# mesnico/ALADIN

Measured on AMD Instinct MI355X. Metric: alignment image-text pairs/sec (BxB scores, triplet loss fwd+bwd) at B=256/GPU,R=34,T=50,D=768, higher is better.
Workload: dtype f16

## Files before the change

### aladin_amd/csrc/align_bwd.hip

```cpp
#include "../../include/aladin_hip.h"
#include "bwd_common.hpp"
#include "gemm_core.hpp"
#include "hinge_common.hpp"
#include "small_heads_common.hpp"

#define NO_GRAD 255

using BwdWs = PairWs<uint8_t>;

static size_t bwd_base_bytes(int Bi, int Bc, int T) {
  if (Bi < 1 || Bc < 1 || T < 2) return 0;
  return pair_ws_layout<uint8_t>(Bi, Bc, T - 1, nullptr, nullptr);
}

struct DenseWs { void* xm; void* xe; void* y; float* E; uint8_t* flags; void* rows; };
static size_t dense_ws_layout(const aladin_align_geom* gs, char* base, DenseWs* ws) {
  auto up = [](size_t v) { return (v + 255) / 256 * 256; };
  size_t off = 0;
  if (ws) ws->xm = base + off;
  off += up((size_t)gs->xm_bytes);
  if (ws) ws->xe = base + off;
  off += up((size_t)gs->xe_bytes + 16);
  if (ws) ws->y = base + off;
  off += up((size_t)gs->y_bytes);
// ... 99 lines not shown
      f32x16 acc;
#pragma unroll
      for (int r = 0; r < 16; ++r) acc[r] = 0.f;
      float ss = 0.f;
      if (vec) {
        for (int u = 0; u < D / 8; ++u) {
          const float4 a = *reinterpret_cast<const float4*>(xr + 8 * u + 4 * h);
          const float4 b = *reinterpret_cast<const float4*>(yr + 8 * u + 4 * h);
          ss += a.x * a.x + a.y * a.y + a.z * a.z + a.w * a.w;
          acc = __builtin_amdgcn_mfma_f32_32x32x2f32(a.x, b.x, acc, 0, 0, 0);
          acc = __builtin_amdgcn_mfma_f32_32x32x2f32(a.y, b.y, acc, 0, 0, 0);
          acc = __builtin_amdgcn_mfma_f32_32x32x2f32(a.z, b.z, acc, 0, 0, 0);
          acc = __builtin_amdgcn_mfma_f32_32x32x2f32(a.w, b.w, acc, 0, 0, 0);
        }
      } else {
        for (int k = 0; k < D; k += 2) {
          const int kk = k + h;
          const float a = kk < D ? xr[kk] : 0.f;
          const float b = kk < D ? yr[kk] : 0.f;
          ss += a * a;
          acc = __builtin_amdgcn_mfma_f32_32x32x2f32(a, b, acc, 0, 0, 0);
        }
      }
      ss += __shfl_xor(ss, 32, 64);
#pragma unroll
      for (int r = 0; r < 16; ++r) {
        const int row = cos_tile_row(r, h);
        const float inv = cos_tile_inv_norm(ss, row);
        blk[tm * 32 + row][tn * 32 + l5] = acc[r] * inv;
      }
    }
    __syncthreads();
    uint8_t* trow = table + ((int64_t)i * Bc + j) * tstride;
    for (int w = threadIdx.x; w < tstride; w += blockDim.x) {
      uint8_t res = NO_GRAD;
      if (w < Lj && Li > 0) {
        float best = blk[0][w];
        int arg = 0;
        for (int r = 1; r < Li; ++r) {
          const float v = blk[r][w];
          if (v > best) { best = v; arg = r; }
        }
        if (!(Li < Rq && best <= 0.f)) res = (uint8_t)arg;
      }
      trow[w] = res;
    }
  }
}

#define CAND_MAX 4096
#define AMBIG_MARGIN 2.2e-3f

using PairCfg = GemmCfg<2, 2, 1, 1>;
#define PAIR_STAGES 3

#ifdef ALADIN_DIAG
__device__ unsigned long long g_pair_probe[8 * 1024];
extern "C" __attribute__((visibility("default"))) int aladin_debug_read_pair_probe(unsigned long long* host_out, int n_blocks) {
  if (!host_out || n_blocks < 1 || n_blocks > 1024) { aladin_set_error("debug_read_pair_probe: bad argument"); return ALADIN_ERR_ARG; }
  if (hipMemcpyFromSymbol(host_out, HIP_SYMBOL(g_pair_probe), (size_t)n_blocks * 64) != hipSuccess) { aladin_set_error("debug_read_pair_probe: copy failed"); return ALADIN_ERR_HIP; }
  return ALADIN_OK;
}
#define PAIR_STAMP(k) do { if (threadIdx.x == 0 && blockIdx.x < 1024) g_pair_probe[8 * blockIdx.x + (k)] = __builtin_amdgcn_s_memrealtime(); } while (0)
#else
#define PAIR_STAMP(k) do { } while (0)
#endif

struct PairHinge {
  const float* S; int64_t ld; float margin; const float* val; const int* arg; float* loss; float* dS; int B; int n_pair_blocks;
  float* dST;
};
template <int SRC>
__global__ __launch_bounds__(256) void bwd_pair_argmax16_kernel(
    const half_t* __restrict__ xm, const half_t* __restrict__ xe, const half_t* __restrict__ y, int Dp, int mrows, int rem,
    int tpad, int xe_rows, int y_rows, const float* __restrict__ im, int64_t im_sb, int64_t im_sr,
    const int32_t* __restrict__ im_len, const float* __restrict__ s, int64_t s_sb, int64_t s_st,
    const int32_t* __restrict__ s_len, int Bc, int Rq, int Tq, int D, const int* __restrict__ counter,
    const int* __restrict__ pairs, uint8_t* __restrict__ table, int tstride, int x_tail,
    int y_tail, PairHinge hf, SmallFin sf) {
  if constexpr (SRC == 2) {
    if ((int)blockIdx.x >= hf.n_pair_blocks) {
      heads_small_finish_body((int)blockIdx.x - hf.n_pair_blocks, (int)gridDim.x - hf.n_pair_blocks, sf);
      return;
    }
  }
  if constexpr (SRC == 1) {
    if ((int)blockIdx.x >= hf.n_pair_blocks) {
      hinge_finish_body((int)blockIdx.x - hf.n_pair_blocks, (int)gridDim.x - hf.n_pair_blocks, hf.S, hf.ld, hf.B, hf.margin, 1,
                        hf.val, hf.arg, hf.loss, hf.dS, nullptr, nullptr, hf.dST);
      return;
    }
  }
  extern __shared__ __attribute__((aligned(16))) char pair_smem[];
  uint8_t* cand_w = reinterpret_cast<uint8_t*>(pair_smem);
  uint8_t* cand_r = cand_w + CAND_MAX;
  static_assert(2 * CAND_MAX <= PAIR_STAGES * PairCfg::STAGE_BYTES, "candidate list must fit in the ring");
  __shared__ float top_b1[2][64], top_b2[2][64];
  __shared__ int top_a1[2][64];
  __shared__ int ncand;
  __shared__ uint8_t word_amb[64], word_res[64];
  __shared__ unsigned long long word_key[64];
  const int wave = threadIdx.x >> 6, lane = threadIdx.x & 63;
  const int h = lane >> 5, l5 = lane & 31;
  const int wm = wave >> 1, wn = wave & 1;
  PAIR_STAMP(0);
  const int count = SRC != 0 ? 3 * hf.B : *counter;
  const int stride = SRC != 0 ? hf.n_pair_blocks : (int)gridDim.x;
  const int per_xcd = (count + 7) >> 3;
  for (int b = blockIdx.x; b < 8 * per_xcd; b += stride) {
    const int p = (b & 7) * per_xcd + (b >> 3);
    if (p >= count) continue;
    int i, j;
    if constexpr (SRC != 0) {
      const int q = p / 3, t = p - 3 * q, B = hf.B;
      auto row_val = [&](int v) { return SRC == 1 ? hf.val[v] : sf.st[(int64_t)v * SB_ST + 8]; };
      auto row_arg = [&](int v) { return SRC == 1 ? hf.arg[v] : __float_as_int(sf.st[(int64_t)v * SB_ST + 9]); };
      const float vr = row_val(q), vc = row_val(B + q);
      bool active;
      if (t == 0) { i = q; j = q; active = vr > 0.f || vc > 0.f; }
      else if (t == 1) { i = q; j = row_arg(q); active = vr > 0.f; }
      else {
        i = q; j = q; active = vc > 0.f;
        if (active) { i = row_arg(B + q); active = !(row_val(i) > 0.f && row_arg(i) == q); }
      }
      if (!active) continue;
    } else {
      i = pairs[p] / Bc; j = pairs[p] % Bc;
    }
    int Li = im_len[i] - 1 - x_tail; Li = Li < 0 ? 0 : (Li > Rq ? Rq : Li);
    int Lj = s_len[j] - 1 - y_tail; Lj = Lj < 0 ? 0 : (Lj > Tq ? Tq : Lj);
    __syncthreads();
    if (Li + Lj >= 0) PAIR_STAMP(1);
    if (threadIdx.x == 0) ncand = 0;
    if (threadIdx.x < 64) { word_amb[threadIdx.x] = 0; word_res[threadIdx.x] = NO_GRAD; word_key[threadIdx.x] = 0ull; }
    const int M = mrows, win = 64 - M;
    const bool side = rem > 0 && win > 0;
    int be = 0;
    if (side) be = i * rem < xe_rows - win ? i * rem : xe_rows - win;
    const int eo = side ? i * rem - be : 0;
    const int64_t yrow = (int64_t)j * tpad;
    const int64_t by = yrow < (int64_t)y_rows - 64 ? yrow : (int64_t)y_rows - 64;
    const int co = (int)(yrow - by);
    const half_t* pa1 = xm + (int64_t)i * M * Dp;
    const half_t* pa2 = side ? xe + (int64_t)be * Dp : pa1;
    f32x16 acc[1][1];
#pragma unroll
    for (int r = 0; r < 16; ++r) acc[0][0][r] = 0.f;
    uint32_t skip = 0;
    {
      const int wv = __builtin_amdgcn_readfirstlane(threadIdx.x >> 6);
      const int w0 = 32 + 8 * wv - M;
      if (w0 >= 0 && (!side || w0 + 8 <= eo || w0 >= eo + rem)) skip |= 2u;
      if (8 * wv + 8 <= co || 8 * wv >= co + tpad) skip |= 4u;
      if (32 + 8 * wv + 8 <= co || 32 + 8 * wv >= co + tpad) skip |= 8u;
    }
    gemm_mainloop<PairCfg, PAIR_STAGES>(pa1, y + by * Dp, Dp, Dp / 64, pair_smem, acc, pa2, M, skip);
    PAIR_STAMP(2);
    const int wcol = wn * 32 + l5;
    const int wd = wcol - co;
    const bool wvalid = wd >= 0 && wd < Lj && Li > 0;
    float b1 = -INFINITY, b2 = -INFINITY;
    int a1 = 255;
    auto region_of = [&](int r) {
      const int gr = wm * 32 + (r & 3) + 8 * (r >> 2) + 4 * h;
      const int d = gr - M - eo;
      const int sreg = ((unsigned)d < (unsigned)rem) ? M + d : 255;
      return gr < M ? gr : sreg;
    };
#pragma unroll
    for (int r = 0; r < 16; ++r) {
      const int reg = region_of(r);
      const float v = reg < Li ? acc[0][0][r] : -INFINITY;
      const bool first = v > b1;
      b2 = first ? b1 : (v > b2 ? v : b2);
      a1 = first ? reg : a1;
      b1 = first ? v : b1;
    }
#define TOP2_MERGE(ob1, oa1, ob2)                                                              \
    do {                                                                                       \
      if ((ob1) > b1 || ((ob1) == b1 && (oa1) < a1)) { b2 = fmaxf(b1, (ob2)); b1 = (ob1); a1 = (oa1); } \
      else b2 = fmaxf(b2, (ob1));                                                              \
    } while (0)
    {
      const float ob1 = lane_xor32(b1), ob2 = lane_xor32(b2);
      const int oa1 = lane_xor32(a1);
      TOP2_MERGE(ob1, oa1, ob2);
    }
    if (h == 0) { top_b1[wm][wcol] = b1; top_b2[wm][wcol] = b2; top_a1[wm][wcol] = a1; }
    __syncthreads();
    {
      const float ob1 = top_b1[wm ^ 1][wcol], ob2 = top_b2[wm ^ 1][wcol];
      const int oa1 = top_a1[wm ^ 1][wcol];
      TOP2_MERGE(ob1, oa1, ob2);
    }
#undef TOP2_MERGE
    if (wvalid) {
      const bool amb = (b1 - b2 < AMBIG_MARGIN) || (Li < Rq && fabsf(b1) < AMBIG_MARGIN);
      if (wm == 0 && h == 0) {
        word_amb[wd] = amb ? 1 : 0;
        word_res[wd] = (Li < Rq && b1 <= 0.f) ? NO_GRAD : (uint8_t)a1;
      }
      if (amb) {
        unsigned close = 0;
#pragma unroll
        for (int r = 0; r < 16; ++r) close |= (unsigned)(region_of(r) < Li && acc[0][0][r] > b1 - AMBIG_MARGIN) << r;
        while (close) {
          const int r = __ffs((int)close) - 1; close &= close - 1;
          const int slot = atomicAdd(&ncand, 1);
          cand_w[slot] = (uint8_t)wd;
// ... 299 lines not shown
    return ALADIN_ERR_ARG;
  }
  if (!set_ok(&im) || !set_ok(&s) || !dS || !workspace) { aladin_set_error("align_bwd: null argument"); return ALADIN_ERR_ARG; }
  if (g->Bi < 1 || g->Bc < 1 || g->R < 2 + g->x_tail || g->T < 2 + g->y_tail || g->D < 1 || ld_dS < g->Bc) { aladin_set_error("align_bwd: bad sizes"); return ALADIN_ERR_ARG; }
  if (bwd_Rq(g) > PA_MAXR - 2 || bwd_Rq(g) >= NO_GRAD || bwd_Tq(g) > PA_MAXT) { aladin_set_error("align_bwd: at most %d regions / %d words", PA_MAXR - 2, PA_MAXT); return ALADIN_ERR_UNSUPPORTED; }
  if (g->D % 4 != 0 || g->D > 1024 || im.stride_b % 4 || im.stride_r % 4 || s.stride_b % 4 || s.stride_r % 4 || ((uintptr_t)im.data & 15) || ((uintptr_t)s.data & 15)) {
    aladin_set_error("align_bwd: needs D %% 4 == 0, D <= 1024 and 16-byte aligned rows (D=%d)", g->D);
    return ALADIN_ERR_UNSUPPORTED;
  }
  if (pr.pk && g->rem && !pr.pk->xe) { aladin_set_error("align_bwd: packed operands do not belong to this problem"); return ALADIN_ERR_ARG; }
  if ((flags & ALADIN_BWD_OWN_ROW_FP16) && !(flags & ALADIN_BWD_PARTNERS_FP16)) { aladin_set_error("align_bwd: ALADIN_BWD_OWN_ROW_FP16 goes with ALADIN_BWD_PARTNERS_FP16"); return ALADIN_ERR_ARG; }
  if ((flags & ALADIN_BWD_PARTNERS_FP16) && (!pr.pk || !pr.pk->rnorm || g->split)) {
    aladin_set_error("align_bwd: ALADIN_BWD_PARTNERS_FP16 needs the forward's fp16 packed operands (xm, xe, y, rnorm) and their geometry");
    return ALADIN_ERR_ARG;
  }
  return ALADIN_OK;
}

int aladin_internal_compact_pairs(const float* dS, int64_t ld, int Bi, int Bc, int* counter, int* pairs, const char* entry, hipStream_t st) {
  if (hipMemsetAsync(counter, 0, 256, st) != hipSuccess) { aladin_set_error("%s: memset failed", entry); return ALADIN_ERR_HIP; }
  const int64_t n = (int64_t)Bi * Bc;
  int grid = (int)((n + 255) / 256); if (grid > 1024) grid = 1024;
  hipLaunchKernelGGL(bwd_compact_kernel, dim3(grid), dim3(256), 0, st, dS, ld, Bi, Bc, counter, pairs);
  return aladin_check_launch("bwd_compact_kernel");
}

template <int SRC>
static int launch_pair16(const BwdProblem& pr, const int* counter, const int* pairs, uint8_t* table, int grid, const PairHinge& hf,
                         const SmallFin& sf, const char* what) {
  const aladin_align_geom* g = pr.g;
  hipLaunchKernelGGL(bwd_pair_argmax16_kernel<SRC>, dim3(grid), dim3(256), (size_t)PAIR_STAGES * PairCfg::STAGE_BYTES, pr.st,
                     (const half_t*)pr.pk->xm, (const half_t*)pr.pk->xe, (const half_t*)pr.pk->y, g->Dp, g->mrows, g->rem, g->trows,
                     (int)g->xe_rows, (int)g->y_rows, pr.im.data, pr.im.stride_b, pr.im.stride_r, pr.im.len, pr.s.data, pr.s.stride_b,
                     pr.s.stride_r, pr.s.len, g->Bc, bwd_Rq(g), bwd_Tq(g), g->D, counter, pairs, table, table_stride(bwd_Tq(g)), g->x_tail,
                     g->y_tail, hf, sf);
  return aladin_check_launch(what);
}

static int hinge_table_check(const BwdProblem& pr, const float* S, int64_t ldS, const float* loss, const float* dS, const void* hinge_ws,
                             const void* bwd_workspace, bool small) {
  const aladin_align_geom* g = pr.g;
  if (!S || !loss || !dS || !hinge_ws || g->Bi != g->Bc || ldS < g->Bc) { aladin_set_error("hinge_argmax: bad argument"); return ALADIN_ERR_ARG; }
  if (small && g->Bc > SB_MAX) { aladin_set_error("heads_small: B = %d > %d", g->Bc, SB_MAX); return ALADIN_ERR_UNSUPPORTED; }
  if (int rc = bwd_check(pr, dS, g->Bc, nullptr, nullptr, bwd_workspace, 0)) return rc;
  if (!pr.pair16) { aladin_set_error("hinge_argmax: needs the packed fp16 operands of a class the fp16 pair kernel covers (R' <= 64, <= 64 padded words)"); return ALADIN_ERR_UNSUPPORTED; }
  return ALADIN_OK;
}
static int table_from_small_heads(const BwdProblem& pr, SmallFin sf, const BwdWs& ws) {
  const int B = pr.g->Bc, npb = (3 * B + 7) / 8 * 8;
  const PairHinge hf = {nullptr, 0, 0.f, nullptr, nullptr, nullptr, nullptr, B, npb, nullptr};
  sf.dST = (float*)ws.pairs;
  return launch_pair16<2>(pr, nullptr, nullptr, ws.table, npb + cdiv(B * B, 256), hf, sf, "bwd_pair_argmax16_kernel<small heads>");
}
static int table_from_hinge(const BwdProblem& pr, const float* S, int64_t ldS, float margin, float* loss, float* dS, void* hinge_ws,
                            const BwdWs& ws) {
  const int B = pr.g->Bc;
  if (int rc = aladin_internal_hinge_stats(S, ldS, B, margin, 1, hinge_ws, nullptr, pr.st)) return rc;
  const float* val = (const float*)hinge_ws;
  const int* arg = (const int*)(val + 2 * (size_t)B);
  int npb = (3 * B + 7) / 8 * 8; if (npb > 2048) npb = 2048;
  const int nfin = B < 1024 ? B : 1024;
  const PairHinge hf = {S, ldS, margin, val, arg, loss, dS, B, npb, (float*)ws.pairs};
  return launch_pair16<1>(pr, nullptr, nullptr, ws.table, npb + nfin, hf, SmallFin{}, "bwd_pair_argmax16_kernel<hinge>");
}

static int table_from_list(const BwdProblem& pr, const int* counter, const int* pairs, uint8_t* table) {
  const aladin_align_geom* g = pr.g;
  const int64_t n = (int64_t)g->Bi * g->Bc;
  const int grid = (int)(n < 2048 ? n : 2048);
  if (pr.pair16) return launch_pair16<0>(pr, counter, pairs, table, grid, PairHinge{}, SmallFin{}, "bwd_pair_argmax16_kernel");
  hipLaunchKernelGGL(bwd_pair_argmax_kernel, dim3(grid), dim3(256), 0, pr.st, pr.im.data, pr.im.stride_b, pr.im.stride_r, pr.im.len,
                     pr.s.data, pr.s.stride_b, pr.s.stride_r, pr.s.len, g->Bc, bwd_Rq(g), bwd_Tq(g), g->D, counter, pairs, table,
                     table_stride(bwd_Tq(g)), g->x_tail, g->y_tail);
  return aladin_check_launch("bwd_pair_argmax_kernel");
}

static int table_all_pairs(const BwdProblem& pr, const aladin_align_geom* gs, const DenseWs& dw, const float* dS, int64_t ld_dS, const BwdWs& ws) {
  const aladin_packed pd = {dw.xm, dw.xe, dw.y, nullptr};
  if (int rc = aladin_internal_pack(&pr.im, &pr.s, gs, &pd, pr.st)) return rc;
  if (int rc = aladin_internal_align_argmax(gs, dw.xm, dw.xe, dw.y, dw.E, pr.im.len, pr.s.len, ws.table, table_stride(bwd_Tq(pr.g)), dw.flags, pr.st)) return rc;
  if (hipMemsetAsync(ws.counter, 0, 256, pr.st) != hipSuccess) { aladin_set_error("align_bwd: memset failed"); return ALADIN_ERR_HIP; }
  const int64_t n = (int64_t)pr.g->Bi * pr.g->Bc;
  int grid = (int)((n + 255) / 256); if (grid > 1024) grid = 1024;
  hipLaunchKernelGGL(bwd_compact_flagged_kernel, dim3(grid), dim3(256), 0, pr.st, dS, ld_dS, pr.g->Bi, pr.g->Bc, dw.flags, ws.counter, ws.pairs);
  return aladin_check_launch("bwd_compact_flagged_kernel");
}

template <int NCH>
static void launch_rows(const BwdProblem& pr, const float* dS, int64_t ld_dS, const float* dST, const float* gscale, const uint8_t* table,
                        const aladin_set_grad* d_im, const aladin_set_grad* d_s, const PackedRows& pk, bool p16, bool o16) {
  const aladin_align_geom* g = pr.g;
  const int64_t rows = (int64_t)g->Bi * g->R + (int64_t)g->Bc * g->T;
  auto go = [&](auto kernel) {
    hipLaunchKernelGGL(kernel, dim3((unsigned)((rows + 3) / 4)), dim3(256), 0, pr.st, pr.im.data, pr.im.stride_b, pr.im.stride_r, pr.im.len,
                       pr.s.data, pr.s.stride_b, pr.s.stride_r, pr.s.len, g->Bi, g->Bc, g->R, g->T, g->D, dS, ld_dS, dST, gscale, table,
                       table_stride(bwd_Tq(g)), d_im->data, d_s->data, g->x_tail, g->y_tail, d_im->stride_b, d_im->stride_r, d_s->stride_b,
                       d_s->stride_r, pk);
  };
  const bool full = g->D == 256 * NCH;
  if (full) o16 ? go(bwd_rows_kernel<NCH, true, true, true>) : p16 ? go(bwd_rows_kernel<NCH, true, true, false>) : go(bwd_rows_kernel<NCH, true, false, false>);
  else o16 ? go(bwd_rows_kernel<NCH, false, true, true>) : p16 ? go(bwd_rows_kernel<NCH, false, true, false>) : go(bwd_rows_kernel<NCH, false, false, false>);
}
static int rows_gather(const BwdProblem& pr, const float* dS, int64_t ld_dS, const float* dST, const float* gscale, const uint8_t* table,
                       const aladin_set_grad* d_im, const aladin_set_grad* d_s, int flags) {
  const aladin_align_geom* g = pr.g;
  const bool p16 = (flags & ALADIN_BWD_PARTNERS_FP16) != 0, o16 = (flags & ALADIN_BWD_OWN_ROW_FP16) != 0;
  PackedRows pk = {nullptr, nullptr, nullptr, 0, 0, 0, 0, nullptr, 0, 0};
  if (p16) pk = PackedRows{(const half_t*)pr.pk->xm, (const half_t*)pr.pk->xe, (const half_t*)pr.pk->y, g->Dp, g->mrows, g->rem, g->trows, pr.pk->rnorm, g->xm_rows, g->xm_rows + g->xe_rows};
  switch ((g->D + 255) / 256) {
    case 1: launch_rows<1>(pr, dS, ld_dS, dST, gscale, table, d_im, d_s, pk, p16, o16); break;
    case 2: launch_rows<2>(pr, dS, ld_dS, dST, gscale, table, d_im, d_s, pk, p16, o16); break;
    case 3: launch_rows<3>(pr, dS, ld_dS, dST, gscale, table, d_im, d_s, pk, p16, o16); break;
    default: launch_rows<4>(pr, dS, ld_dS, dST, gscale, table, d_im, d_s, pk, p16, o16); break;
  }
// ... 128 lines not shown
```

### aladin_amd/csrc/gemm_core.hpp

```cpp
#pragma once
#include "common.hpp"

template <int WGM_, int WGN_, int WM_, int WN_, int CT16_ = 2 * WN_, int RT16_ = 2 * WM_>
struct GemmCfg {
  static constexpr int WGM = WGM_, WGN = WGN_, WM = WM_, WN = WN_, CT16 = CT16_, RT16 = RT16_;
  static constexpr int WCOLS = 16 * CT16;
  static constexpr int WROWS = 16 * RT16;
  static constexpr int NWAVES = WGM * WGN;
  static constexpr int THREADS = NWAVES * 64;
  static constexpr int BM = WGM * WROWS;
  static constexpr int BN = WGN * WCOLS;
  static constexpr int ROWS = BM + BN;
  static constexpr int STAGE_BYTES = ROWS * 128;
  static constexpr int CHUNKS = ROWS / 8;
  static constexpr bool EVEN_CHUNKS = CHUNKS % NWAVES == 0;
  static constexpr int CHUNKS_PER_WAVE = (CHUNKS + NWAVES - 1) / NWAVES;
  static constexpr int LDS_BYTES = 2 * STAGE_BYTES;
  static_assert(ROWS % 8 == 0, "stages are filled in 8-row pieces");
};

template <class Cfg>
__device__ __forceinline__ uint32_t stage_lane_offset(int64_t ldk, int wave, int lane) {
  static_assert(Cfg::NWAVES % 2 == 0, "piece parity must be a wave constant");
  const int r = lane >> 3;
// ... 58 lines not shown
    default: asm volatile("s_waitcnt vmcnt(0)" ::: "memory"); break;
  }
}

template <class Cfg, int NS = 2, bool SPREAD = false>
__device__ __forceinline__ void gemm_mainloop(const half_t* __restrict__ a_rows, const half_t* __restrict__ b_rows,
                                              int64_t ldk, int ktiles, char* smem, f32x16 (&acc)[Cfg::WM][Cfg::WN],
                                              const half_t* __restrict__ a_rows2 = nullptr, int a_split = Cfg::BM,
                                              uint32_t skip = 0) {
  static_assert(NS >= 2 && Cfg::CHUNKS_PER_WAVE * (NS - 2) <= 32, "ring too deep for the vmcnt dispatcher");
  static_assert(Cfg::CT16 == 2 * Cfg::WN, "32 x 32 accumulator tiles: whole 32-column units per wave");
  const int n_issued = Cfg::CHUNKS_PER_WAVE - __builtin_popcount(skip);
  const int wave = __builtin_amdgcn_readfirstlane(threadIdx.x >> 6);
  const int lane = threadIdx.x & 63;
  const int wm = wave / Cfg::WGN, wn = wave % Cfg::WGN;
  const uint32_t lane_off = stage_lane_offset<Cfg>(ldk, wave, lane);
  const int a_row0 = wm * Cfg::WM * 32 + (lane & 31);
  const int b_row0 = Cfg::BM + wn * Cfg::WN * 32 + (lane & 31);

#pragma unroll
  for (int st = 0; st < NS - 1; ++st)
    if (st < ktiles) gemm_stage<Cfg>(a_rows, a_rows2, a_split, b_rows, ldk, st, smem + st * Cfg::STAGE_BYTES, wave, lane_off, skip);
  for (int kt = 0; kt < ktiles; ++kt) {
    const int ahead = ktiles - 1 - kt;
    wait_vmcnt(n_issued * (ahead < NS - 2 ? ahead : NS - 2));
    __builtin_amdgcn_s_barrier();
    const char* cur = smem + (kt % NS) * Cfg::STAGE_BYTES;
    const bool refill = kt + NS - 1 < ktiles;
    char* nxt = smem + ((kt + NS - 1) % NS) * Cfg::STAGE_BYTES;
    if (!SPREAD && refill) gemm_stage<Cfg>(a_rows, a_rows2, a_split, b_rows, ldk, kt + NS - 1, nxt, wave, lane_off, skip);
#pragma unroll
    for (int kk = 0; kk < 4; ++kk) {
      half8 af[Cfg::WM], bf[Cfg::WN];
#pragma unroll
      for (int a = 0; a < Cfg::WM; ++a) af[a] = lds_frag(cur, a_row0 + a * 32, kk, lane);
#pragma unroll
      for (int n = 0; n < Cfg::WN; ++n) bf[n] = lds_frag(cur, b_row0 + n * 32, kk, lane);
      if (SPREAD && refill) {
        constexpr int CPW = Cfg::CHUNKS_PER_WAVE;
        if (kk == 0) gemm_stage<Cfg, 0, (CPW + 3) / 4>(a_rows, a_rows2, a_split, b_rows, ldk, kt + NS - 1, nxt, wave, lane_off);
        if (kk == 1) gemm_stage<Cfg, (CPW + 3) / 4, (2 * CPW + 3) / 4>(a_rows, a_rows2, a_split, b_rows, ldk, kt + NS - 1, nxt, wave, lane_off);
        if (kk == 2) gemm_stage<Cfg, (2 * CPW + 3) / 4, (3 * CPW + 3) / 4>(a_rows, a_rows2, a_split, b_rows, ldk, kt + NS - 1, nxt, wave, lane_off);
        if (kk == 3) gemm_stage<Cfg, (3 * CPW + 3) / 4, CPW>(a_rows, a_rows2, a_split, b_rows, ldk, kt + NS - 1, nxt, wave, lane_off);
      }
#pragma unroll
      for (int a = 0; a < Cfg::WM; ++a)
#pragma unroll
        for (int n = 0; n < Cfg::WN; ++n)
          acc[a][n] = __builtin_amdgcn_mfma_f32_32x32x16_f16(af[a], bf[n], acc[a][n], 0, 0, 0);
    }
  }
}

__device__ __forceinline__ half8 lds_frag16(const char* stage, int row, int k32, int lane) {
  const int logical = k32 * 4 + (lane >> 4);
  const int phys = logical ^ ((row >> 1) & 7);
  return *reinterpret_cast<const half8*>(stage + row * 128 + phys * 16);
}

template <class Cfg, bool SPREAD = true, int NS = 2>
__device__ __forceinline__ void gemm_mainloop16(const half_t* __restrict__ a_rows, const half_t* __restrict__ b_rows,
                                                int64_t ldk, int ktiles, char* smem,
                                                f32x4 (&acc)[2 * Cfg::WM][2 * Cfg::WN]) {
  constexpr int RT = 2 * Cfg::WM, CT = 2 * Cfg::WN;
  static_assert(RT == 4, "written for a 64-row wave tile");
  static_assert(Cfg::CT16 == 2 * Cfg::WN && Cfg::RT16 == 2 * Cfg::WM && Cfg::EVEN_CHUNKS, "whole 32-row / 32-column units per wave");
  constexpr int CPW = Cfg::CHUNKS_PER_WAVE;
  const int wave = __builtin_amdgcn_readfirstlane(threadIdx.x >> 6);
  const int lane = threadIdx.x & 63;
  const int wm = wave / Cfg::WGN, wn = wave % Cfg::WGN;
  const uint32_t lane_off = stage_lane_offset<Cfg>(ldk, wave, lane);
  const int a_row0 = wm * Cfg::WM * 32 + (lane & 15);
  const int b_row0 = Cfg::BM + wn * Cfg::WN * 32 + (lane & 15);

  static_assert(NS >= 2 && CPW * (NS - 2) <= 32, "ring too deep for the vmcnt dispatcher");
  constexpr int LEAD = NS - 1;
#pragma unroll
  for (int st = 0; st < LEAD; ++st)
    if (st < ktiles) gemm_stage<Cfg>(a_rows, nullptr, Cfg::BM, b_rows, ldk, st, smem + st * Cfg::STAGE_BYTES, wave, lane_off);
  for (int kt = 0; kt < ktiles; ++kt) {
    if constexpr (NS == 2) asm volatile("s_waitcnt vmcnt(0)" ::: "memory");
    else {
      const int ahead = ktiles - 1 - kt;
      wait_vmcnt(CPW * (ahead < NS - 2 ? ahead : NS - 2));
    }
    __builtin_amdgcn_s_barrier();
    const char* cur = smem + (kt % NS) * Cfg::STAGE_BYTES;
    const bool refill = kt + LEAD < ktiles;
    char* nxt = smem + ((kt + LEAD) % NS) * Cfg::STAGE_BYTES;
    if (!SPREAD && refill) gemm_stage<Cfg>(a_rows, nullptr, Cfg::BM, b_rows, ldk, kt + LEAD, nxt, wave, lane_off);

    static_assert(CT == 12, "three clusters of four column tiles");
    half8 a[RT], bA[4], bB[4];
    bA[0] = lds_frag16(cur, b_row0, 0, lane);
#pragma unroll
    for (int rt = 0; rt < RT; ++rt) a[rt] = lds_frag16(cur, a_row0 + rt * 16, 0, lane);
#pragma unroll
    for (int j = 1; j < 4; ++j) bA[j] = lds_frag16(cur, b_row0 + j * 16, 0, lane);
#pragma unroll
    for (int k32 = 0; k32 < 2; ++k32) {
#pragma unroll
      for (int j = 0; j < 4; ++j) bB[j] = lds_frag16(cur, b_row0 + (4 + j) * 16, k32, lane);
      if (SPREAD && refill) {
        if (k32 == 1) gemm_stage<Cfg, (6 * CPW) / 10, (8 * CPW) / 10>(a_rows, nullptr, Cfg::BM, b_rows, ldk, kt + LEAD, nxt, wave, lane_off);
      }
      __builtin_amdgcn_sched_barrier(0);
// ... 137 lines not shown
```

### aladin_amd/csrc/hinge_common.hpp

```cpp
#pragma once
#include "common.hpp"

__device__ __forceinline__ float block_sum(float v, float* red) {
  v = wave_sum(v);
  const int wave = threadIdx.x >> 6, lane = threadIdx.x & 63;
  __syncthreads();
  if (lane == 0) red[wave] = v;
  __syncthreads();
  float t = 0.f;
  for (int w = 0; w < (int)(blockDim.x >> 6); ++w) t += red[w];
  return t;
}

__device__ __forceinline__ void hinge_finish_body(int vblock, int nblocks, const float* __restrict__ S, int64_t ld, int B,
                                                  float margin, int max_violation, const float* __restrict__ val,
                                                  const int* __restrict__ arg, float* __restrict__ loss,
                                                  float* __restrict__ dS, int* __restrict__ pairs,
                                                  int* __restrict__ pair_count, float* __restrict__ dST = nullptr) {
  __shared__ float red[4];
  if (vblock == 0) {
    float rs = 0.f, cs = 0.f;
    for (int t = threadIdx.x; t < B; t += blockDim.x) { rs += val[t]; cs += val[B + t]; }
    rs = block_sum(rs, red);
    cs = block_sum(cs, red);
    if (threadIdx.x == 0) *loss = rs + cs;
  }
  if (dS == nullptr && pairs == nullptr) return;
  const int lane = threadIdx.x & 63;
  for (int i = vblock; i < B; i += nblocks) {
    const float rv = val[i], di = S[(int64_t)i * ld + i];
    const int ra = arg[i];
    for (int j0 = 0; j0 < B; j0 += blockDim.x) {
      const int j = j0 + threadIdx.x;
      float g = 0.f;
      if (j < B) {
        if (max_violation) {
          if (i == j) g = -(float)((rv > 0.f) + (val[B + i] > 0.f));
          else g = (float)((rv > 0.f && ra == j) + (val[B + j] > 0.f && arg[B + j] == i));
        } else {
          if (i == j) g = -(float)(ra + arg[B + i]);
          else {
            const float s = S[(int64_t)i * ld + j];
            g = (float)((margin + s - di > 0.f) + (margin + s - S[(int64_t)j * ld + j] > 0.f));
          }
        }
        if (dS) dS[(int64_t)i * B + j] = g;
        if (dST) dST[(int64_t)j * B + i] = g;
      }
      if (pairs) {
        __shared__ int wcnt[4];
        __shared__ int wbase;
        const unsigned long long mask = __ballot(g != 0.f);
        const int wv = threadIdx.x >> 6;
        __syncthreads();
        if (lane == 0) wcnt[wv] = __popcll(mask);
        __syncthreads();
        if (threadIdx.x == 0) {
          const int tot = wcnt[0] + wcnt[1] + wcnt[2] + wcnt[3];
          wbase = tot ? atomicAdd(pair_count, tot) : 0;
        }
        __syncthreads();
        if (g != 0.f) {
          int base = wbase;
          for (int q = 0; q < wv; ++q) base += wcnt[q];
          pairs[base + __popcll(mask & ((1ull << lane) - 1))] = i * B + j;
        }
      }
    }
  }
}

int aladin_internal_hinge_stats(const float* S, int64_t ldS, int B, float margin, int max_violation, void* workspace,
                                int* pair_count, hipStream_t st);
```

### aladin_amd/csrc/losses.hip

```cpp
#include "../../include/aladin_hip.h"
#include "common.hpp"
#include "hinge_common.hpp"
#include "sgemm_tile.hpp"

__device__ __forceinline__ float block_max(float v, float* red) {
  v = wave_max(v);
  const int wave = threadIdx.x >> 6, lane = threadIdx.x & 63;
  __syncthreads();
  if (lane == 0) red[wave] = v;
  __syncthreads();
  float t = red[0];
  for (int w = 1; w < (int)(blockDim.x >> 6); ++w) t = fmaxf(t, red[w]);
  return t;
}
__device__ __forceinline__ void block_argmax(float& v, int& idx, float* redv, int* redi) {
  wave_argmax(v, idx);
  const int wave = threadIdx.x >> 6, lane = threadIdx.x & 63;
  __syncthreads();
  if (lane == 0) { redv[wave] = v; redi[wave] = idx; }
  __syncthreads();
  v = redv[0]; idx = redi[0];
  for (int w = 1; w < (int)(blockDim.x >> 6); ++w)
    if (redv[w] > v || (redv[w] == v && redi[w] < idx)) { v = redv[w]; idx = redi[w]; }
}

__global__ __launch_bounds__(256) void hinge_stats_kernel(const float* __restrict__ S, int64_t ld, int B, float margin,
                                                          int max_violation, float* __restrict__ val,
                                                          int* __restrict__ arg, int* __restrict__ pair_count) {
  __shared__ float redv[4];
  __shared__ int redi[4];
  const int b = blockIdx.x;
  if (b == 0 && threadIdx.x == 0 && pair_count) *pair_count = 0;
  const bool is_row = b < B;
  const int q = is_row ? b : b - B;
  const float diag = S[(int64_t)q * ld + q];
  float best = 0.f, sum = 0.f;
  int besti = 0x7fffffff, cnt = 0;
  for (int t = threadIdx.x; t < B; t += blockDim.x) {
    const float s = is_row ? S[(int64_t)q * ld + t] : S[(int64_t)t * ld + q];
    float c = fmaxf(margin + s - diag, 0.f);
    if (t == q) c = 0.f;
    if (c > best || (c == best && t < besti)) { best = c; besti = t; }
    sum += c;
    cnt += (c > 0.f);
  }
  if (max_violation) {
    block_argmax(best, besti, redv, redi);
    if (threadIdx.x == 0) { val[b] = best; arg[b] = besti; }
  } else {
    sum = block_sum(sum, redv);
    const float fc = block_sum((float)cnt, redv);
    if (threadIdx.x == 0) { val[b] = sum; arg[b] = (int)fc; }
  }
}

__global__ __launch_bounds__(256) void hinge_finish_kernel(const float* __restrict__ S, int64_t ld, int B, float margin,
                                                           int max_violation, const float* __restrict__ val,
                                                           const int* __restrict__ arg, float* __restrict__ loss,
                                                           float* __restrict__ dS, int* __restrict__ pairs,
                                                           int* __restrict__ pair_count) {
  hinge_finish_body((int)blockIdx.x, (int)gridDim.x, S, ld, B, margin, max_violation, val, arg, loss, dS, pairs, pair_count);
}

extern "C" size_t aladin_hinge_workspace_bytes(int B) { return (size_t)(B > 0 ? B : 0) * 16 + 256; }

int aladin_internal_hinge_stats(const float* S, int64_t ldS, int B, float margin, int max_violation, void* workspace,
                                int* pair_count, hipStream_t st) {
  float* val = (float*)workspace;
  int* arg = (int*)(val + 2 * (size_t)B);
  hipLaunchKernelGGL(hinge_stats_kernel, dim3(2 * B), dim3(256), 0, st, S, ldS, B, margin, max_violation, val, arg, pair_count);
  return aladin_check_launch("hinge_stats_kernel");
}

static int hinge_impl(const float* S, int64_t ldS, int B, float margin, int max_violation, float* loss, float* dS,
                      int32_t* pairs, int32_t* pair_count, void* workspace, void* stream) {
  if (!S || !loss || !workspace || B < 1 || ldS < B || (pairs && !pair_count)) { aladin_set_error("hinge: bad argument (B=%d ldS=%lld)", B, (long long)ldS); return ALADIN_ERR_ARG; }
  float* val = (float*)workspace;
  int* arg = (int*)(val + 2 * (size_t)B);
  hipStream_t st = (hipStream_t)stream;
  int rc = aladin_internal_hinge_stats(S, ldS, B, margin, max_violation, workspace, pairs ? pair_count : nullptr, st);
  if (rc) return rc;
  const int grid = (dS || pairs) ? (B < 2048 ? B : 2048) : 1;
  hipLaunchKernelGGL(hinge_finish_kernel, dim3(grid < 1 ? 1 : grid), dim3(256), 0, st, S, ldS, B, margin, max_violation, val,
                     arg, loss, dS, pairs, pair_count);
  return aladin_check_launch("hinge_finish_kernel");
}

extern "C" int aladin_hinge_fwd_bwd(const float* S, int64_t ldS, int B, float margin, int max_violation, float* loss,
                                    float* dS, void* workspace, void* stream) {
  return hinge_impl(S, ldS, B, margin, max_violation, loss, dS, nullptr, nullptr, workspace, stream);
}

extern "C" int aladin_hinge_fused(const float* S, int64_t ldS, int B, float margin, int max_violation, float* loss,
                                  float* dS, int32_t* pairs, int32_t* pair_count, void* workspace, void* stream) {
  return hinge_impl(S, ldS, B, margin, max_violation, loss, dS, pairs, pair_count, workspace, stream);
}

__global__ __launch_bounds__(256) void listnet_stats_kernel(const float* __restrict__ T, int64_t ldt,
// ... 151 lines not shown
```

Measured before the change: 331.5 million.

## Fuse hinge statistics into pair kernel and deepen register-prefetch GEMM mainloop

Removes the separate hinge_stats launch for B<=256. Pair blocks now recompute each row or column argmax on the fly, and the finish blocks rebuild the column stats themselves in LDS. The pair GEMM mainloop is replaced with a register-staged prefetch six tiles deep over a two-stage LDS ring, and the kernel gets launch_bounds with a minimum of 3 blocks. The intent is to save a kernel launch and global round trip and to hide load latency. In exchange, stats are scanned redundantly across blocks, register pressure rises, and every finish block rescans the whole S matrix.

Result: slower. 291.1 million (-12.2%).

```diff
diff --git a/aladin_amd/csrc/align_bwd.hip b/aladin_amd/csrc/align_bwd.hip
--- a/aladin_amd/csrc/align_bwd.hip
+++ b/aladin_amd/csrc/align_bwd.hip
@@ -175,7 +175,8 @@
 #define AMBIG_MARGIN 2.2e-3f
 
 using PairCfg = GemmCfg<2, 2, 1, 1>;
-#define PAIR_STAGES 3
+#define PAIR_STAGES 2
+#define PAIR_DEPTH 6
 
 #ifdef ALADIN_DIAG
 __device__ unsigned long long g_pair_probe[8 * 1024];
@@ -194,13 +195,14 @@
   float* dST;
 };
 template <int SRC>
-__global__ __launch_bounds__(256) void bwd_pair_argmax16_kernel(
+__global__ __launch_bounds__(256, 3) void bwd_pair_argmax16_kernel(
     const half_t* __restrict__ xm, const half_t* __restrict__ xe, const half_t* __restrict__ y, int Dp, int mrows, int rem,
     int tpad, int xe_rows, int y_rows, const float* __restrict__ im, int64_t im_sb, int64_t im_sr,
     const int32_t* __restrict__ im_len, const float* __restrict__ s, int64_t s_sb, int64_t s_st,
     const int32_t* __restrict__ s_len, int Bc, int Rq, int Tq, int D, const int* __restrict__ counter,
     const int* __restrict__ pairs, uint8_t* __restrict__ table, int tstride, int x_tail,
     int y_tail, PairHinge hf, SmallFin sf) {
+  extern __shared__ __attribute__((aligned(16))) char pair_smem[];
   if constexpr (SRC == 2) {
     if ((int)blockIdx.x >= hf.n_pair_blocks) {
       heads_small_finish_body((int)blockIdx.x - hf.n_pair_blocks, (int)gridDim.x - hf.n_pair_blocks, sf);
@@ -209,12 +211,15 @@
   }
   if constexpr (SRC == 1) {
     if ((int)blockIdx.x >= hf.n_pair_blocks) {
-      hinge_finish_body((int)blockIdx.x - hf.n_pair_blocks, (int)gridDim.x - hf.n_pair_blocks, hf.S, hf.ld, hf.B, hf.margin, 1,
-                        hf.val, hf.arg, hf.loss, hf.dS, nullptr, nullptr, hf.dST);
+      if (hf.val == nullptr)
+        hinge_finish_fused_body((int)blockIdx.x - hf.n_pair_blocks, (int)gridDim.x - hf.n_pair_blocks, hf.S, hf.ld, hf.B, hf.margin,
+                                hf.loss, hf.dS, hf.dST, pair_smem);
+      else
+        hinge_finish_body((int)blockIdx.x - hf.n_pair_blocks, (int)gridDim.x - hf.n_pair_blocks, hf.S, hf.ld, hf.B, hf.margin, 1,
+                          hf.val, hf.arg, hf.loss, hf.dS, nullptr, nullptr, hf.dST);
       return;
     }
   }
-  extern __shared__ __attribute__((aligned(16))) char pair_smem[];
   uint8_t* cand_w = reinterpret_cast<uint8_t*>(pair_smem);
   uint8_t* cand_r = cand_w + CAND_MAX;
   static_assert(2 * CAND_MAX <= PAIR_STAGES * PairCfg::STAGE_BYTES, "candidate list must fit in the ring");
@@ -223,6 +228,8 @@
   __shared__ int ncand;
   __shared__ uint8_t word_amb[64], word_res[64];
   __shared__ unsigned long long word_key[64];
+  __shared__ float stat_v[4];
+  __shared__ int stat_i[4];
   const int wave = threadIdx.x >> 6, lane = threadIdx.x & 63;
   const int h = lane >> 5, l5 = lane & 31;
   const int wm = wave >> 1, wn = wave & 1;
@@ -236,15 +243,26 @@
     int i, j;
     if constexpr (SRC != 0) {
       const int q = p / 3, t = p - 3 * q, B = hf.B;
-      auto row_val = [&](int v) { return SRC == 1 ? hf.val[v] : sf.st[(int64_t)v * SB_ST + 8]; };
-      auto row_arg = [&](int v) { return SRC == 1 ? hf.arg[v] : __float_as_int(sf.st[(int64_t)v * SB_ST + 9]); };
-      const float vr = row_val(q), vc = row_val(B + q);
+      auto stat = [&](int v, float& val, int& arg) {
+        if constexpr (SRC == 1) {
+          if (hf.val == nullptr) hinge_line_argmax(hf.S, hf.ld, B, hf.margin, v < B, v < B ? v : v - B, val, arg, stat_v, stat_i);
+          else { val = hf.val[v]; arg = hf.arg[v]; }
+        } else { val = sf.st[(int64_t)v * SB_ST + 8]; arg = __float_as_int(sf.st[(int64_t)v * SB_ST + 9]); }
+      };
+      float vr = 0.f, vc = 0.f;
+      int ar = 0, ac = 0;
+      if (t != 2) stat(q, vr, ar);
+      if (t != 1) stat(B + q, vc, ac);
       bool active;
       if (t == 0) { i = q; j = q; active = vr > 0.f || vc > 0.f; }
-      else if (t == 1) { i = q; j = row_arg(q); active = vr > 0.f; }
+      else if (t == 1) { i = q; j = ar; active = vr > 0.f; }
       else {
         i = q; j = q; active = vc > 0.f;
-        if (active) { i = row_arg(B + q); active = !(row_val(i) > 0.f && row_arg(i) == q); }
+        if (active) {
+          float vi; int ai;
+          i = ac; stat(i, vi, ai);
+          active = !(vi > 0.f && ai == q);
+        }
       }
       if (!active) continue;
     } else {
@@ -277,7 +295,7 @@
       if (8 * wv + 8 <= co || 8 * wv >= co + tpad) skip |= 4u;
       if (32 + 8 * wv + 8 <= co || 32 + 8 * wv >= co + tpad) skip |= 8u;
     }
-    gemm_mainloop<PairCfg, PAIR_STAGES>(pa1, y + by * Dp, Dp, Dp / 64, pair_smem, acc, pa2, M, skip);
+    gemm_mainloop_deep<PairCfg, PAIR_DEPTH>(pa1, y + by * Dp, Dp, Dp / 64, pair_smem, acc, pa2, M, skip);
     PAIR_STAMP(2);
     const int wcol = wn * 32 + l5;
     const int wd = wcol - co;
@@ -683,14 +701,23 @@
   sf.dST = (float*)ws.pairs;
   return launch_pair16<2>(pr, nullptr, nullptr, ws.table, npb + cdiv(B * B, 256), hf, sf, "bwd_pair_argmax16_kernel<small heads>");
 }
+#ifndef HINGE_FUSED_MAX_B
+#define HINGE_FUSED_MAX_B 256
+#endif
 static int table_from_hinge(const BwdProblem& pr, const float* S, int64_t ldS, float margin, float* loss, float* dS, void* hinge_ws,
                             const BwdWs& ws) {
   const int B = pr.g->Bc;
-  if (int rc = aladin_internal_hinge_stats(S, ldS, B, margin, 1, hinge_ws, nullptr, pr.st)) return rc;
-  const float* val = (const float*)hinge_ws;
-  const int* arg = (const int*)(val + 2 * (size_t)B);
+  static_assert(hinge_fused_lds_bytes(HINGE_FUSED_MAX_B) <= (size_t)PAIR_STAGES * PairCfg::STAGE_BYTES, "the fused statistics live in the ring");
+  const bool fused = B <= HINGE_FUSED_MAX_B;
+  const float* val = nullptr;
+  const int* arg = nullptr;
+  if (!fused) {
+    if (int rc = aladin_internal_hinge_stats(S, ldS, B, margin, 1, hinge_ws, nullptr, pr.st)) return rc;
+    val = (const float*)hinge_ws;
+    arg = (const int*)(val + 2 * (size_t)B);
+  }
   int npb = (3 * B + 7) / 8 * 8; if (npb > 2048) npb = 2048;
-  const int nfin = B < 1024 ? B : 1024;
+  const int nfin = fused ? cdiv(B, HINGE_FUSED_ROWS) : (B < 1024 ? B : 1024);
   const PairHinge hf = {S, ldS, margin, val, arg, loss, dS, B, npb, (float*)ws.pairs};
   return launch_pair16<1>(pr, nullptr, nullptr, ws.table, npb + nfin, hf, SmallFin{}, "bwd_pair_argmax16_kernel<hinge>");
 }
diff --git a/aladin_amd/csrc/gemm_core.hpp b/aladin_amd/csrc/gemm_core.hpp
--- a/aladin_amd/csrc/gemm_core.hpp
+++ b/aladin_amd/csrc/gemm_core.hpp
@@ -134,6 +134,90 @@
   }
 }
 
+typedef uint32_t u32x4 __attribute__((ext_vector_type(4)));
+template <class Cfg, int DEPTH, int D, int C = 0>
+__device__ __forceinline__ void deep_fetch(u32x4 (&buf)[DEPTH][Cfg::CHUNKS_PER_WAVE], const __amdgpu_buffer_rsrc_t (&rs)[Cfg::CHUNKS_PER_WAVE],
+                                           uint32_t voff) {
+  if constexpr (C < Cfg::CHUNKS_PER_WAVE) {
+    buf[D][C] = __builtin_amdgcn_raw_buffer_load_b128(rs[C], voff, 0, 0);
+    deep_fetch<Cfg, DEPTH, D, C + 1>(buf, rs, voff);
+  }
+}
+template <class Cfg, int DEPTH, int D, int C = 0>
+__device__ __forceinline__ void deep_store(const u32x4 (&buf)[DEPTH][Cfg::CHUNKS_PER_WAVE], char* stage, int wave, int lane) {
+  if constexpr (C < Cfg::CHUNKS_PER_WAVE) {
+    *reinterpret_cast<u32x4*>(stage + (wave + C * Cfg::NWAVES) * 1024 + lane * 16) = buf[D][C];
+    deep_store<Cfg, DEPTH, D, C + 1>(buf, stage, wave, lane);
+  }
+}
+__device__ __forceinline__ uint32_t deep_voff(uint32_t lane_off, int kt, int ktiles) {
+  return kt < ktiles ? lane_off + (uint32_t)kt * 128u : 0x80000000u;
+}
+template <class Cfg, int DEPTH, int D = 0>
+__device__ __forceinline__ void deep_prologue(u32x4 (&buf)[DEPTH][Cfg::CHUNKS_PER_WAVE], const __amdgpu_buffer_rsrc_t (&rs)[Cfg::CHUNKS_PER_WAVE],
+                                              uint32_t lane_off, int ktiles) {
+  if constexpr (D < DEPTH) {
+    deep_fetch<Cfg, DEPTH, D>(buf, rs, deep_voff(lane_off, D, ktiles));
+    deep_prologue<Cfg, DEPTH, D + 1>(buf, rs, lane_off, ktiles);
+  }
+}
+template <class Cfg, int DEPTH, int D = 0>
+__device__ __forceinline__ void deep_steps(u32x4 (&buf)[DEPTH][Cfg::CHUNKS_PER_WAVE], const __amdgpu_buffer_rsrc_t (&rs)[Cfg::CHUNKS_PER_WAVE],
+                                           uint32_t lane_off, int kt0, int ktiles, char* smem, int wave, int lane, int a_row0, int b_row0,
+                                           f32x16 (&acc)[Cfg::WM][Cfg::WN]) {
+  if constexpr (D < DEPTH) {
+    const int kt = kt0 + D;
+    char* cur = smem + (kt & 1) * Cfg::STAGE_BYTES;
+    deep_store<Cfg, DEPTH, D>(buf, cur, wave, lane);
+    deep_fetch<Cfg, DEPTH, D>(buf, rs, deep_voff(lane_off, kt + DEPTH, ktiles));
+    asm volatile("s_waitcnt lgkmcnt(0)" ::: "memory");
+    __builtin_amdgcn_s_barrier();
+#pragma unroll
+    for (int kk = 0; kk < 4; ++kk) {
+      half8 af[Cfg::WM], bf[Cfg::WN];
+#pragma unroll
+      for (int a = 0; a < Cfg::WM; ++a) af[a] = lds_frag(cur, a_row0 + a * 32, kk, lane);
+#pragma unroll
+      for (int n = 0; n < Cfg::WN; ++n) bf[n] = lds_frag(cur, b_row0 + n * 32, kk, lane);
+#pragma unroll
+      for (int a = 0; a < Cfg::WM; ++a)
+#pragma unroll
+        for (int n = 0; n < Cfg::WN; ++n)
+          acc[a][n] = __builtin_amdgcn_mfma_f32_32x32x16_f16(af[a], bf[n], acc[a][n], 0, 0, 0);
+    }
+    deep_steps<Cfg, DEPTH, D + 1>(buf, rs, lane_off, kt0, ktiles, smem, wave, lane, a_row0, b_row0, acc);
+  }
+}
+
+template <class Cfg, int DEPTH>
+__device__ __forceinline__ void gemm_mainloop_deep(const half_t* __restrict__ a_rows, const half_t* __restrict__ b_rows,
+                                                   int64_t ldk, int ktiles, char* smem, f32x16 (&acc)[Cfg::WM][Cfg::WN],
+                                                   const half_t* __restrict__ a_rows2 = nullptr, int a_split = Cfg::BM,
+                                                   uint32_t skip = 0) {
+  static_assert(Cfg::EVEN_CHUNKS && Cfg::CT16 == 2 * Cfg::WN && Cfg::RT16 == 2 * Cfg::WM, "whole 32 x 32 tiles, pieces dealt evenly");
+  constexpr int CPW = Cfg::CHUNKS_PER_WAVE;
+  const int wave = __builtin_amdgcn_readfirstlane(threadIdx.x >> 6);
+  const int lane = threadIdx.x & 63;
+  const int wm = wave / Cfg::WGN, wn = wave % Cfg::WGN;
+  const uint32_t lane_off = stage_lane_offset<Cfg>(ldk, wave, lane);
+  const int a_row0 = wm * Cfg::WM * 32 + (lane & 31);
+  const int b_row0 = Cfg::BM + wn * Cfg::WN * 32 + (lane & 31);
+  __amdgpu_buffer_rsrc_t rs[CPW];
+#pragma unroll
+  for (int c = 0; c < CPW; ++c) {
+    const int row0 = (wave + c * Cfg::NWAVES) * 8;
+    const half_t* base;
+    if (row0 < Cfg::BM) base = (row0 < a_split) ? a_rows + (int64_t)row0 * ldk : a_rows2 + (int64_t)(row0 - a_split) * ldk;
+    else base = b_rows + (int64_t)(row0 - Cfg::BM) * ldk;
+    const int bytes = ((skip >> c) & 1u) ? 0 : (int)(ldk * 16);
+    rs[c] = __builtin_amdgcn_make_buffer_rsrc(const_cast<half_t*>(base), 0, bytes, 0x00020000);
+  }
+  u32x4 buf[DEPTH][CPW];
+  deep_prologue<Cfg, DEPTH>(buf, rs, lane_off, ktiles);
+  for (int kt0 = 0; kt0 < ktiles; kt0 += DEPTH)
+    deep_steps<Cfg, DEPTH>(buf, rs, lane_off, kt0, ktiles, smem, wave, lane, a_row0, b_row0, acc);
+}
+
 __device__ __forceinline__ half8 lds_frag16(const char* stage, int row, int k32, int lane) {
   const int logical = k32 * 4 + (lane >> 4);
   const int phys = logical ^ ((row >> 1) & 7);
diff --git a/aladin_amd/csrc/hinge_common.hpp b/aladin_amd/csrc/hinge_common.hpp
--- a/aladin_amd/csrc/hinge_common.hpp
+++ b/aladin_amd/csrc/hinge_common.hpp
@@ -10,6 +10,52 @@
   float t = 0.f;
   for (int w = 0; w < (int)(blockDim.x >> 6); ++w) t += red[w];
   return t;
+}
+__device__ __forceinline__ void block_argmax(float& v, int& idx, float* redv, int* redi) {
+  wave_argmax(v, idx);
+  const int wave = threadIdx.x >> 6, lane = threadIdx.x & 63;
+  __syncthreads();
+  if (lane == 0) { redv[wave] = v; redi[wave] = idx; }
+  __syncthreads();
+  v = redv[0]; idx = redi[0];
+  for (int w = 1; w < (int)(blockDim.x >> 6); ++w)
+    if (redv[w] > v || (redv[w] == v && redi[w] < idx)) { v = redv[w]; idx = redi[w]; }
+}
+
+__device__ __forceinline__ float hinge_cost(float margin, float s, float diag, bool on_diag) {
+  const float c = fmaxf(margin + s - diag, 0.f);
+  return on_diag ? 0.f : c;
+}
+struct HingeLine { float best, sum; int besti, cnt; };
+__device__ __forceinline__ HingeLine hinge_line_scan(const float* __restrict__ S, int64_t ld, int B, float margin, bool is_row, int q) {
+  const float diag = S[(int64_t)q * ld + q];
+  HingeLine h = {0.f, 0.f, 0x7fffffff, 0};
+  for (int t = threadIdx.x; t < B; t += blockDim.x) {
+    const float s = is_row ? S[(int64_t)q * ld + t] : S[(int64_t)t * ld + q];
+    const float c = hinge_cost(margin, s, diag, t == q);
+    if (c > h.best || (c == h.best && t < h.besti)) { h.best = c; h.besti = t; }
+    h.sum += c;
+    h.cnt += (c > 0.f);
+  }
+  return h;
+}
+__device__ __forceinline__ void hinge_line_argmax(const float* __restrict__ S, int64_t ld, int B, float margin, bool is_row, int q,
+                                                  float& val, int& arg, float* redv, int* redi) {
+  const HingeLine h = hinge_line_scan(S, ld, B, margin, is_row, q);
+  val = h.best; arg = h.besti;
+  block_argmax(val, arg, redv, redi);
+}
+
+__device__ __forceinline__ void hinge_loss_sum(const float* rowv, const float* colv, int B, float* red, float* __restrict__ loss) {
+  float rs = 0.f, cs = 0.f;
+  for (int t = threadIdx.x; t < B; t += blockDim.x) { rs += rowv[t]; cs += colv[t]; }
+  rs = block_sum(rs, red);
+  cs = block_sum(cs, red);
+  if (threadIdx.x == 0) *loss = rs + cs;
+}
+__device__ __forceinline__ float hinge_mv_grad(int i, int j, float rv, int ra, float cv_i, float cv_j, int ca_j) {
+  if (i == j) return -(float)((rv > 0.f) + (cv_i > 0.f));
+  return (float)((rv > 0.f && ra == j) + (cv_j > 0.f && ca_j == i));
 }
 
 __device__ __forceinline__ void hinge_finish_body(int vblock, int nblocks, const float* __restrict__ S, int64_t ld, int B,
@@ -18,13 +64,7 @@
                                                   float* __restrict__ dS, int* __restrict__ pairs,
                                                   int* __restrict__ pair_count, float* __restrict__ dST = nullptr) {
   __shared__ float red[4];
-  if (vblock == 0) {
-    float rs = 0.f, cs = 0.f;
-    for (int t = threadIdx.x; t < B; t += blockDim.x) { rs += val[t]; cs += val[B + t]; }
-    rs = block_sum(rs, red);
-    cs = block_sum(cs, red);
-    if (threadIdx.x == 0) *loss = rs + cs;
-  }
+  if (vblock == 0) hinge_loss_sum(val, val + B, B, red, loss);
   if (dS == nullptr && pairs == nullptr) return;
   const int lane = threadIdx.x & 63;
   for (int i = vblock; i < B; i += nblocks) {
@@ -35,8 +75,7 @@
       float g = 0.f;
       if (j < B) {
         if (max_violation) {
-          if (i == j) g = -(float)((rv > 0.f) + (val[B + i] > 0.f));
-          else g = (float)((rv > 0.f && ra == j) + (val[B + j] > 0.f && arg[B + j] == i));
+          g = hinge_mv_grad(i, j, rv, ra, val[B + i], val[B + j], arg[B + j]);
         } else {
           if (i == j) g = -(float)(ra + arg[B + i]);
           else {
@@ -70,5 +109,103 @@
   }
 }
 
+#define HINGE_FUSED_ROWS 4
+static constexpr size_t hinge_fused_lds_bytes(int B) { return (size_t)B * 12 + 4 * 256 * 8; }
+
+template <bool ROWS>
+__device__ __forceinline__ void hinge_all_columns(const float* __restrict__ S, int64_t ld, int B, float margin, float* cval, int* carg,
+                                                  float* rval, float* pv, int* pi) {
+  const int wave = threadIdx.x >> 6, lane = threadIdx.x & 63;
+  const bool vec = (ld % 4 == 0) && (((uintptr_t)S & 15) == 0);
+  for (int c0 = 0; c0 < B; c0 += 256) {
+    const int col = c0 + 4 * lane;
+    float dg[4], best[4];
+    int besti[4];
+#pragma unroll
+    for (int u = 0; u < 4; ++u) {
+      dg[u] = col + u < B ? S[(int64_t)(col + u) * ld + col + u] : 0.f;
+      best[u] = 0.f; besti[u] = 0x7fffffff;
+    }
+    for (int r0 = wave; r0 < B; r0 += 16) {
+      float s[4][4];
+#pragma unroll
+      for (int k = 0; k < 4; ++k) {
+        const int r = r0 + 4 * k;
+        const float* row = S + (int64_t)r * ld;
+#pragma unroll
+        for (int u = 0; u < 4; ++u) s[k][u] = 0.f;
+        if (r >= B) continue;
+        if (vec && col + 3 < B) { const float4 v = *reinterpret_cast<const float4*>(row + col); s[k][0] = v.x; s[k][1] = v.y; s[k][2] = v.z; s[k][3] = v.w; }
+        else {
+#pragma unroll
+          for (int u = 0; u < 4; ++u) if (col + u < B) s[k][u] = row[col + u];
+        }
+      }
+#pragma unroll
+      for (int k = 0; k < 4; ++k) {
+        const int r = r0 + 4 * k;
+        if (r >= B) continue;
+        float m = 0.f;
+        const float dr = ROWS ? S[(int64_t)r * ld + r] : 0.f;
+#pragma unroll
+        for (int u = 0; u < 4; ++u) {
+          if (col + u < B) {
+            const float c = hinge_cost(margin, s[k][u], dg[u], r == col + u);
+            if (c > best[u] || (c == best[u] && r < besti[u])) { best[u] = c; besti[u] = r; }
+            if (ROWS) m = fmaxf(m, hinge_cost(margin, s[k][u], dr, r == col + u));
+          }
+        }
+        if (ROWS) {
+          m = wave_max(m);
+          if (lane == 0) rval[r] = c0 ? fmaxf(rval[r], m) : m;
+        }
+      }
+    }
+#pragma unroll
+    for (int u = 0; u < 4; ++u) { pv[wave * 256 + 4 * lane + u] = best[u]; pi[wave * 256 + 4 * lane + u] = besti[u]; }
+    __syncthreads();
+    if (c0 + (int)threadIdx.x < B) {
+      float v = pv[threadIdx.x];
+      int a = pi[threadIdx.x];
+      for (int w = 1; w < 4; ++w) {
+        const float ov = pv[w * 256 + threadIdx.x];
+        const int oa = pi[w * 256 + threadIdx.x];
+        if (ov > v || (ov == v && oa < a)) { v = ov; a = oa; }
+      }
+      cval[c0 + threadIdx.x] = v; carg[c0 + threadIdx.x] = a;
+    }
+    __syncthreads();
+  }
+}
+
+__device__ __forceinline__ void hinge_finish_fused_body(int vblock, int nblocks, const float* __restrict__ S, int64_t ld, int B,
+                                                        float margin, float* __restrict__ loss, float* __restrict__ dS,
+                                                        float* __restrict__ dST, char* smem) {
+  __shared__ float red[4];
+  __shared__ int redi[4];
+  float* cval = reinterpret_cast<float*>(smem);
+  int* carg = reinterpret_cast<int*>(cval + B);
+  float* rval = reinterpret_cast<float*>(carg + B);
+  float* pv = rval + B;
+  int* pi = reinterpret_cast<int*>(pv + 4 * 256);
+  if (vblock == 0) {
+    hinge_all_columns<true>(S, ld, B, margin, cval, carg, rval, pv, pi);
+    hinge_loss_sum(rval, cval, B, red, loss);
+  } else {
+    hinge_all_columns<false>(S, ld, B, margin, cval, carg, rval, pv, pi);
+  }
+  for (int i = vblock; i < B; i += nblocks) {
+    float rv;
+    int ra;
+    hinge_line_argmax(S, ld, B, margin, true, i, rv, ra, red, redi);
+    const float cv_i = cval[i];
+    for (int j = threadIdx.x; j < B; j += blockDim.x) {
+      const float g = hinge_mv_grad(i, j, rv, ra, cv_i, cval[j], carg[j]);
+      dS[(int64_t)i * B + j] = g;
+      if (dST) dST[(int64_t)j * B + i] = g;
+    }
+  }
+}
+
 int aladin_internal_hinge_stats(const float* S, int64_t ldS, int B, float margin, int max_violation, void* workspace,
                                 int* pair_count, hipStream_t st);
diff --git a/aladin_amd/csrc/losses.hip b/aladin_amd/csrc/losses.hip
--- a/aladin_amd/csrc/losses.hip
+++ b/aladin_amd/csrc/losses.hip
@@ -13,16 +13,6 @@
   for (int w = 1; w < (int)(blockDim.x >> 6); ++w) t = fmaxf(t, red[w]);
   return t;
 }
-__device__ __forceinline__ void block_argmax(float& v, int& idx, float* redv, int* redi) {
-  wave_argmax(v, idx);
-  const int wave = threadIdx.x >> 6, lane = threadIdx.x & 63;
-  __syncthreads();
-  if (lane == 0) { redv[wave] = v; redi[wave] = idx; }
-  __syncthreads();
-  v = redv[0]; idx = redi[0];
-  for (int w = 1; w < (int)(blockDim.x >> 6); ++w)
-    if (redv[w] > v || (redv[w] == v && redi[w] < idx)) { v = redv[w]; idx = redi[w]; }
-}
 
 __global__ __launch_bounds__(256) void hinge_stats_kernel(const float* __restrict__ S, int64_t ld, int B, float margin,
                                                           int max_violation, float* __restrict__ val,
@@ -33,17 +23,10 @@
   if (b == 0 && threadIdx.x == 0 && pair_count) *pair_count = 0;
   const bool is_row = b < B;
   const int q = is_row ? b : b - B;
-  const float diag = S[(int64_t)q * ld + q];
-  float best = 0.f, sum = 0.f;
-  int besti = 0x7fffffff, cnt = 0;
-  for (int t = threadIdx.x; t < B; t += blockDim.x) {
-    const float s = is_row ? S[(int64_t)q * ld + t] : S[(int64_t)t * ld + q];
-    float c = fmaxf(margin + s - diag, 0.f);
-    if (t == q) c = 0.f;
-    if (c > best || (c == best && t < besti)) { best = c; besti = t; }
-    sum += c;
-    cnt += (c > 0.f);
-  }
+  const HingeLine h = hinge_line_scan(S, ld, B, margin, is_row, q);
+  float best = h.best, sum = h.sum;
+  int besti = h.besti;
+  const int cnt = h.cnt;
   if (max_violation) {
     block_argmax(best, besti, redv, redi);
     if (threadIdx.x == 0) { val[b] = best; arg[b] = besti; }
```
